# xandergos/terrain-diffusion

Hardware: AMD Instinct MI355X
Metric: terrain megapixels/sec (decoded) at fixed steps, 30m model (higher is better)
Workload: dtype bf16; 1 GPU; BASELINE configs[2]: terrain-diffusion-30m base U-Net, 8x8 tile grid (stride 32, 288x288 latents) with overlap blending, 20 steps, 64 windows batched per solver step; edm_steps=20, parallelism=1 independent streams (one process per GPU, no data-path collective)

## Files before the change

### terrain_diffusion_amd/csrc/conv_common.h

```cpp
#pragma once
#include "td_device.h"

#ifdef TD_ABLATE_BLOAD
#define TD_ABL_BLOAD(X)
#else
#define TD_ABL_BLOAD(X) X
#endif
#ifdef TD_ABLATE_BARRIER
#define TD_ABL_BARRIER(X)
#else
#define TD_ABL_BARRIER(X) X
#endif
#ifdef TD_ABLATE_BSTORE
#define TD_ABL_BSTORE(X)
#else
#define TD_ABL_BSTORE(X) X
#endif

#define TD_SWZ(r) (((r) >> 1) & 7)

namespace td {

typedef __bf16 bf16x8 __attribute__((ext_vector_type(8)));
typedef __bf16 bf16x4 __attribute__((ext_vector_type(4)));
// ... 244 lines not shown
            const f32x2 r[4] = {{(float)ra[0], (float)ra[1]}, {(float)ra[2], (float)ra[3]}, {(float)rb[0], (float)rb[1]}, {(float)rb[2], (float)rb[3]}};
#pragma unroll
            for (int q = 0; q < 4; ++q) v[q] = v[q] + rs * r[q];
        }
        if (clip > 0.f) {
#pragma unroll
            for (int q = 0; q < 4; ++q) v[q] = f32x2{__builtin_amdgcn_fmed3f(v[q].x, -clip, clip), __builtin_amdgcn_fmed3f(v[q].y, -clip, clip)};
        }
    }
    const hx4 ha = {(T)v[0].x, (T)v[0].y, (T)v[1].x, (T)v[1].y};
    const hx4 hb = {(T)v[2].x, (T)v[2].y, (T)v[3].x, (T)v[3].y};
    const f32x2 f[4] = {{(float)ha[0], (float)ha[1]}, {(float)ha[2], (float)ha[3]}, {(float)hb[0], (float)hb[1]}, {(float)hb[2], (float)hb[3]}};
    if (want_ss) {
        f32x2 s2 = f[0] * f[0];
#pragma unroll
        for (int q = 1; q < 4; ++q) s2 = f[q] * f[q] + s2;
        ss += s2.x + s2.y;
    }
    {
        const u32x2 pa = __builtin_bit_cast(u32x2, ha), pb = __builtin_bit_cast(u32x2, hb);
        unsigned a0 = pa[0], a1 = pa[1], b0 = pb[0], b1 = pb[1];
        swap_halves(a0, b0); swap_halves(a1, b1);
        o = u32x4{a0, a1, b0, b1};
    }
    if (want_o2) {
        f32x2 g[4];
#pragma unroll
        for (int q = 0; q < 4; ++q) g[q] = silu_k2(f[q], k_o2);
        const hx4 ga = {(T)g[0].x, (T)g[0].y, (T)g[1].x, (T)g[1].y}, gb = {(T)g[2].x, (T)g[2].y, (T)g[3].x, (T)g[3].y};
        const u32x2 qa = __builtin_bit_cast(u32x2, ga), qb = __builtin_bit_cast(u32x2, gb);
        unsigned c0 = qa[0], c1 = qa[1], d0 = qb[0], d1 = qb[1];
        swap_halves(c0, d0); swap_halves(c1, d1);
        o2 = u32x4{c0, c1, d0, d1};
    }
}

template <int TW, int TPIX>
__device__ __forceinline__ void frag_pixel(int q0, int l31, int& img, int& ty, int& tx) {
#ifndef TD_NO_REMAP
#define TD_REMAP_ON 1
#else
#define TD_REMAP_ON 0
#endif
    if constexpr (TW == 16 && TD_REMAP_ON) {
        const bool g2 = (l31 >= 4 && l31 < 12) || (l31 >= 16 && l31 < 20) || l31 >= 28;
        const int u = g2 ? (l31 < 12 ? l31 - 4 : (l31 < 20 ? l31 - 8 : l31 - 16)) : (l31 < 4 ? l31 : (l31 < 16 ? l31 - 8 : l31 - 12));
        img = q0 / TPIX;
        ty = (q0 % TPIX) / 16 + (g2 ? 1 : 0);
        tx = u;
    } else if constexpr (TW == 8 && TD_REMAP_ON) {
        const bool g2 = (l31 >= 4 && l31 < 12) || (l31 >= 16 && l31 < 20) || l31 >= 28;
        const int u = g2 ? (l31 < 12 ? l31 - 4 : (l31 < 20 ? l31 - 8 : l31 - 16)) : (l31 < 4 ? l31 : (l31 < 16 ? l31 - 8 : l31 - 12));
        img = q0 / TPIX;
        ty = (q0 % TPIX) / 8 + (u >> 2);
        tx = (u & 3) + (g2 ? 4 : 0);
    } else {
        const int q = q0 + l31, r = q % TPIX;
        img = q / TPIX; ty = r / TW; tx = r % TW;
    }
}

}
```

### terrain_diffusion_amd/csrc/engine.hip

```cpp
#include <hip/hip_runtime.h>
#include <math.h>
#include <stdio.h>
#include <string.h>

#include <map>
#include <memory>
#include <string>
#include <vector>
#include <unordered_map>

#include "../../include/td_engine.h"
#include "td_device.h"

#include "conv_igemm.hip"
#include "conv_glds.hip"
#include "conv_glds_wide.hip"
#include "conv_sb.hip"
#include "conv_s16.hip"
#include "conv_fewcout.hip"
#include "small_kernels.hip"
#include "compose_kernels.hip"
#include "attn_mfma.hip"

using namespace td;

#define TD_DISPATCH_T(U, ...)                                                       \
    do {                                                                             \
        if ((U)->dt == TD_DTYPE_BF16) { typedef __bf16 T_; __VA_ARGS__; }            \
        else if ((U)->dt == TD_DTYPE_F16) { typedef _Float16 T_; __VA_ARGS__; }      \
        else { typedef float T_; __VA_ARGS__; }                                      \
    } while (0)

static thread_local std::string g_err;
static int fail(int code, const std::string& msg) { g_err = msg; return code; }
#define HIP_TRY(expr)                                                                                      \
    do {                                                                                                   \
        hipError_t _e = (expr);                                                                            \
        if (_e != hipSuccess) return fail(TD_ERR_HIP, std::string(#expr) + ": " + hipGetErrorString(_e)); \
    } while (0)

static inline uint16_t f2h(float f) {
    _Float16 h = (_Float16)f;
    uint16_t u;
    memcpy(&u, &h, 2);
    return u;
}
static inline uint16_t f2bf(float f) {
    uint32_t u;
    memcpy(&u, &f, 4);
// ... 185 lines not shown
    bool set = false;
    int64_t numel() const { int64_t n = 1; for (int i = 0; i < ndim; ++i) n *= shape[i]; return n; }
};

struct WSeg {
    const std::vector<float>* w = nullptr;
    int cin_tot = 0, cin_off = 0, c_real = 0, c_pad = 0, taps = 9;
    float mul = 1.f;
};
struct ConvWeights {
    std::vector<WSeg> segs;
    int cout = 0, cout_pad = 0;
    Buf packed;
    int ksteps = 0;
    Buf packed_sb;
    size_t packed_bytes = 0;
    Buf packed_s16;
    int sb_n3 = 0, sb_g1 = 0;
};

struct Tensor {
    void* ptr = nullptr;
    int C = 0, cstride = 0, H = 0, W = 0;
    float* sumsq = nullptr;
    int nparts = 0;
};

struct Op {
    enum Kind { CONV, ATTN } kind = CONV;
    ConvParams p;
    bool narrow = false;
    int bn = 64;
    int glds_variant = 0;
    int flavor = 0;
    int sb_mt = 2, sb_nt = 2;
    int cvec_off = -1;
    double k_alg = 0.0;
    int out_C = 0, out_H = 0, out_W = 0;
    const void* qkv = nullptr; void* att = nullptr; int tokens = 0, C = 0;
    void* attn_ws = nullptr;
    std::string label;
};

struct Plan {
    int N = 0, H = 0, W = 0;
    std::vector<Op> ops;
    std::vector<Buf> bufs;
    void* xin = nullptr;
    float* F = nullptr;
    float* partial = nullptr;
    Buf x, m1, m2, xt, cond, emb, cvec, tsteps;
    int cvec_rows = 0;
    int cvec_written = 0;
    hipGraphExec_t graph = nullptr;
    std::vector<float> graph_sigmas;
    float graph_sigma_data = 0.f;
    int graph_solver_order = 0;
    int graph_lof = -1;
    int graph_fuse = -1;
    int graph_stop = -2;
    const void* graph_guide = nullptr;
    const void* graph_guide_cvec = nullptr;
    float graph_gscale = 0.f;
    float graph_alpha = 1.f;
    std::vector<float> graph_cs;
    size_t bytes = 0;
// ... 297 lines not shown
            if ((rc = mk(n + ".conv_res1", b.cout, s1))) return rc;
        }
        if (b.attn) {
            if ((rc = mk(n + ".attn_qkv", 3 * b.cout, {seg(n + ".attn_qkv.weight", 1.f, b.cout, 0, b.cout, 1, 1.f)}))) return rc;
            if ((rc = mk(n + ".attn_proj", b.cout, {seg(n + ".attn_proj.weight", 1.f, b.cout, 0, b.cout, 1, kMixNew)}))) return rc;
        }
        return TD_OK;
    };
    for (auto& b : u->enc) if ((rc = do_block(b))) return rc;
    for (auto& b : u->dec) if ((rc = do_block(b))) return rc;
    if ((rc = mk("out_conv", u->cfg.out_channels, {seg("out_conv.weight", out_gain, u->final_c, 0, u->final_c, 9, 1.f)}))) return rc;
    for (auto& p : u->params) { p.data.clear(); p.data.shrink_to_fit(); }
    u->folded.clear();
    HIP_TRY(hipDeviceSynchronize());
    u->finalized = true;
    return TD_OK;
}

static int new_buf(Plan& pl, size_t bytes, void** out) {
    Buf b(new DevBuf());
    HIP_TRY(b->alloc(bytes, true));
    *out = b->p;
    pl.bytes += b->bytes;
    pl.bufs.push_back(std::move(b));
    return TD_OK;
}

struct SegSpec { const Tensor* t; int C; int taps; int resample; int xform; float scale; };

static int build_plan(td_unet* u, int N, int H, int W, Plan** out, int lane = 0) {
    static const char* const kPlanOptions[] = {"batch_invariant", "glds", "splitk", "producer_act", "glds_min_wgs", "glds_variant", "glds_bn",
                                               "glds_splitk", "glds_splitk_max", "glds_splitk_min_groups", "splitk_target_wgs",
                                               "bn128_min_wgs", "attn_mfma", "glds_splitk_from_groups", "glds_bn64", "glds_small_max_groups", "glds_round_aware", "walk_alternate", "glds_tiny", "glds_dma1x1", "splitk_weighted",
                                               "sb", "sb_target_wgs", "sb_mt", "sb_nt", "sb_order", "sb_max_glds_wgs", "sb_splitk", "sb_splitk_wgs", "sb_splitk_max", "s16", "s16_min_wgs", "sb_m4", "glds_wide", "glds_wide_min_wgs", "glds_wide_tail", "glds_wide_persist", "fewcout"};
    std::string key = std::to_string(N) + "_" + std::to_string(H) + "_" + std::to_string(W);
    for (const char* o : kPlanOptions) key += "_" + std::to_string((long long)u->eng->option(o, -7));
    if (lane) key += "_lane" + std::to_string(lane);
    auto it = u->plans.find(key);
    if (it != u->plans.end()) { it->second->last_use = ++u->use_clock; *out = it->second.get(); return TD_OK; }
    if (N < 1 || N > 1023 || H > 1023 || W > 1023) return fail(TD_ERR_ARG, "batch/size out of range");
    const int down = 1 << (u->cfg.n_levels - 1);
    if (H % down || W % down) return fail(TD_ERR_ARG, "H and W must be divisible by 2^(levels-1)");
    {
        const size_t budget = (size_t)u->eng->option("plan_cache_mb", 65536) << 20;
        const size_t max_plans = (size_t)u->eng->option("plan_cache_max", 12);
        size_t total = 0;
        for (auto& kv : u->plans) total += kv.second->bytes;
        while (!u->plans.empty() && (total > budget || u->plans.size() >= max_plans)) {
            auto victim = u->plans.begin();
            for (auto jt = u->plans.begin(); jt != u->plans.end(); ++jt) if (jt->second->last_use < victim->second->last_use) victim = jt;
            HIP_TRY(hipStreamSynchronize(u->eng->stream));
            total -= victim->second->bytes;
            u->plans.erase(victim);
        }
    }
    std::unique_ptr<Plan> plp(new Plan());
    Plan& pl = *plp;
    pl.N = N; pl.H = H; pl.W = W;
    const size_t es = u->esize();
    const int chunk = u->chunk;
    const bool use_splitk = u->eng->option("splitk", 1) != 0;
    const int64_t splitk_target = u->eng->option("splitk_target_wgs", 512);
    const int64_t bn128_min = u->eng->option("bn128_min_wgs", 128);
    int rc;
    size_t partial_bytes = 0;

    auto new_tensor = [&](int C, int h, int w, bool want_sumsq, int nparts, Tensor* t) -> int {
// ... 62 lines not shown
            if (u->bf16 && bn2 && u->eng->option("glds", 1) && (inv || sb_takes || mt2 * (cw.cout_pad / bn2) >= u->eng->option("glds_min_wgs", 8))) {
                op.flavor = 2; op.bn = bn2; op.glds_variant = variant;
                int TH2 = variant ? 8 : (op.narrow ? 8 : 16);
                const int NIMG2 = op.narrow ? (variant ? 2 : 4) : 1;
                p.tiles_x = (w + TW2 - 1) / TW2; p.tiles_y = (h + TH2 - 1) / TH2; p.img_groups = (N + NIMG2 - 1) / NIMG2;
                p.n_ntiles = cw.cout_pad / bn2; p.ksplit = 1;
                const int64_t wgs = mt2 * p.n_ntiles, slots = variant ? 512 : 256;
                const bool may_split = !inv && use_splitk && u->eng->option("glds_splitk", 1) && wgs * 2 <= slots;
                if (may_split && kgroups >= u->eng->option("glds_splitk_from_groups", 2))
                    p.ksplit = (int)std::min<int64_t>(std::min<int64_t>(u->eng->option("glds_splitk_max", 32), kgroups / std::max<int64_t>(1, u->eng->option("glds_splitk_min_groups", 1))), slots / wgs);
                if (may_split && !op.narrow && variant == 1 && u->eng->option("glds_tiny", 0) != 0) {
                    const int64_t wgs_tiny = tiles(4, 1) * (cw.cout_pad / 64);
                    if (wgs_tiny <= 384) {
                        op.glds_variant = 2; op.bn = 64; TH2 = 4;
                        p.tiles_y = (h + TH2 - 1) / TH2; p.n_ntiles = cw.cout_pad / 64;
                        p.ksplit = (int)std::max<int64_t>(1, std::min<int64_t>(std::min<int64_t>(kgroups, u->eng->option("glds_splitk_max", 32)), 384 / wgs_tiny));
                    }
                }
                {
                    const int64_t wmode = u->eng->option("glds_wide", 1);
                    const int bnw = cw.cout_pad % 96 == 0 ? 96 : (cw.cout_pad % 64 == 0 ? 64 : 0);
                    const int64_t tmode = u->eng->option("glds_wide_tail", 1);
                    bool pure3 = true;
                    for (const SegSpec& sg : segs) if (sg.taps != 9 && (sg.xform != 0 || tmode == 0 || (tmode == 1 && bnw != 64))) pure3 = false;
                    const int64_t wgs_w = bnw ? tiles(16, 1) * (cw.cout_pad / bnw) : 0;
                    if (wmode != 0 && !inv && fv < 0 && fbn == 0 && !op.narrow && p.ksplit == 1 && bnw && !out_f32 && (cw.cout & 7) == 0 && p.nseg <= 3 && (pure3 || wmode == 2) &&
                        (wmode == 2 || wgs_w >= u->eng->option("glds_wide_min_wgs", 384))) {
                        op.glds_variant = 3; op.bn = bnw;
                        p.tiles_x = (w + 15) / 16; p.tiles_y = (h + 15) / 16; p.img_groups = N; p.n_ntiles = cw.cout_pad / bnw;
                        bool tail3 = false;
                        for (const SegSpec& sg : segs) if (sg.taps != 9) tail3 = true;
                        if (u->eng->option("glds_wide_persist", 0) != 0 && bnw == 64 && !tail3 && (h & 15) == 0 && (w & 15) == 0 && cw.cout == cw.cout_pad)
                            p.persist = conv_wide_persist_grid((long long)p.tiles_x * p.tiles_y * N * p.n_ntiles, 2 * std::max(1, u->eng->n_cus));
                    }
                }
                if (op.flavor == 2 && sb_takes && op.glds_variant != 3) {
                    {
                        const int TWs = op.narrow ? 8 : 16;
                        auto th_of = [&](int mt) { return op.narrow ? (mt == 2 ? 8 : 4) : (mt == 4 ? 8 : mt == 2 ? 4 : 2); };
                        auto sb_wgs = [&](int mt, int nt) { return (int64_t)((w + TWs - 1) / TWs) * ((h + th_of(mt) - 1) / th_of(mt)) * N * (cw.cout_pad / (32 * nt)); };
                        const int64_t target = u->eng->option("sb_target_wgs", 160);
                        int mt = 1, nt = 1, ks = 1;
                        if (!op.narrow && u->eng->option("sb_m4", 0) != 0 && sb_wgs(2, 2) >= target && sb_wgs(4, 1) >= target) { mt = 4; nt = 1; }
                        else if (sb_wgs(2, 2) >= target) { mt = 2; nt = 2; } else if (sb_wgs(2, 1) >= target) { mt = 2; nt = 1; }
                        else if (use_splitk && u->eng->option("sb_splitk", 1) != 0 && sb_wgs(2, 1) * 2 <= u->eng->option("sb_splitk_wgs", 224)) {
                            mt = 2; nt = 1;
                            ks = (int)std::min<int64_t>(std::min<int64_t>(kgroups, u->eng->option("sb_splitk_max", 16)), (u->eng->option("sb_splitk_wgs", 224) + sb_wgs(2, 1) / 2) / sb_wgs(2, 1));
                        }
                        const int64_t fmt = u->eng->option("sb_mt", 0), fnt = u->eng->option("sb_nt", 0);
                        if (fmt == 1 || fmt == 2 || (fmt == 4 && !op.narrow)) { mt = (int)fmt; ks = 1; }
                        if (fnt == 1 || fnt == 2) { nt = (int)fnt; ks = 1; if (mt == 4 && fnt == 2 && fmt != 4) mt = 2; }
                        if (mt == 4) nt = 1;
                        const int64_t s16_mode = u->eng->option("s16", 1);
                        const int64_t wgs16 = sb_wgs(2, 1) * 2;
                        const bool s16 = s16_mode == 2 || (s16_mode == 1 && fmt == 0 && fnt == 0 && sb_wgs(2, 2) < target && sb_wgs(2, 1) < target &&
                                                           wgs16 <= u->eng->option("sb_splitk_wgs", 224) && wgs16 >= u->eng->option("s16_min_wgs", 128));
                        if (s16) {
                            if ((rc = ensure_packed_s16(u, cw))) return rc;
                            op.flavor = 5; op.sb_mt = 2; op.sb_nt = 0; p.ksplit = 1;
                            p.tiles_x = (w + TWs - 1) / TWs; p.tiles_y = (h + th_of(2) - 1) / th_of(2); p.img_groups = N; p.n_ntiles = cw.cout_pad / 16;
                            p.wpack_sb = cw.packed_s16->p; p.sb_n3 = cw.sb_n3;
                        } else {
                        if ((rc = ensure_packed_sb(u, cw))) return rc;
                        op.flavor = 4; op.sb_mt = mt; op.sb_nt = nt; p.ksplit = ks < 1 ? 1 : ks;
                        p.tiles_x = (w + TWs - 1) / TWs; p.tiles_y = (h + th_of(mt) - 1) / th_of(mt); p.img_groups = N; p.n_ntiles = cw.cout_pad / (32 * nt);
                        p.wpack_sb = cw.packed_sb->p; p.sb_n3 = cw.sb_n3;
// ... 255 lines not shown
                if (kind[i / 2] == 0) { u->eng->prof_conv_ms += ms; u->eng->prof_conv_launches++; } else { u->eng->prof_other_ms += ms; u->eng->prof_other_launches++; }
            }
            for (auto e : evs) (void)hipEventDestroy(e);
        }
    } fin{u, evs, ev_kind, ev_label, ev_flop, st};
    for (auto& op : pl.ops) {
        if (op.kind == Op::ATTN) {
            mark();
            if (op.attn_ws) {
                const int Hh = op.C / 64, L = op.tokens;
                size_t qn, kn, vn;
                attn_workspace_elems(pl.N, Hh, L, L, 64, &qn, &kn, &vn);
                __bf16 *Qp = (__bf16*)op.attn_ws, *Kp = Qp + qn, *Vt = Kp + kn;
                const __bf16* qkv = (const __bf16*)op.qkv;
                const AttnStrides so = {(long)L * op.C, 64L, (long)op.C, 1L};
                hipError_t ea = attn_pack_qkv64<__bf16>(qkv, 3L * op.C, pl.N, Hh, L, 0.125f, Qp, Kp, Vt, st);
                if (ea == hipSuccess) ea = attn_mfma(Qp, Kp, Vt, nullptr, (__bf16*)op.att, so, pl.N, Hh, L, L, 64, st);
                if (ea != hipSuccess) return fail(TD_ERR_HIP, std::string("attention launch: ") + hipGetErrorString(ea));
            } else
            TD_DISPATCH_T(u, hipLaunchKernelGGL(attn_kernel<T_>, dim3(pl.N, op.C / 64), dim3(256), 0, st, (const T_*)op.qkv, (T_*)op.att, op.tokens, op.C));
            mark(); if (prof) { ev_kind.push_back(1); ev_label.push_back(op.label); ev_flop.push_back(0.0); }
            HIP_TRY(hipGetLastError());
            continue;
        }
        ConvParams p = op.p;
        if (op.cvec_off >= 0) p.cvec = cbase + op.cvec_off;
        if (fuse && &op == &pl.ops.back()) {
            p.epi = EPI_DPM_STEP; p.dpm_x = (float*)pl.x->p; p.dpm_m1 = (float*)pl.m1->p; p.dpm_m2 = u->eng->option("solver_order", 2) == 3 ? (float*)pl.m2->p : nullptr; p.dpm_xin = pl.xin; p.dpm_xin_cstride = u->chunk; p.dpm_k = *fuse;
        }
        mark();
        hipError_t e = op.flavor == 6 ? launch_conv_fewcout(p, u->dt, st)
                       : op.flavor == 5 ? launch_conv_s16(p, u->dt, op.narrow, st)
                       : op.flavor == 4 ? launch_conv_sb(p, u->dt, op.narrow, op.sb_mt, op.sb_nt, st)
                       : op.flavor == 2 ? (op.glds_variant == 3 ? launch_conv_glds_wide(p, u->dt, op.bn, st) : launch_conv_glds(p, u->dt, op.narrow, op.bn, op.glds_variant, st))
                       : launch_conv(p, u->dt, op.narrow, op.bn, 0, st);
        mark(); if (prof) { ev_kind.push_back(0); char tag[160]; double gf_ = op.k_alg * 2.0 * p.N * p.H * p.W * p.Cout * 1e-9;
            double mb_ = 0.0; const double es_ = (double)u->esize();
            for (int si_ = 0; si_ < p.nseg; ++si_) mb_ += (double)p.N * p.seg[si_].Hs * p.seg[si_].Ws * p.seg[si_].C * es_ + (double)p.seg[si_].C / 64.0 * p.seg[si_].taps * p.CoutPad * 128.0 * (es_ / 2.0);
            if (p.res) mb_ += (double)p.N * p.res_Hs * p.res_Ws * p.Cout * es_;
            const double o1_ = (double)p.N * p.H * p.W * p.Cout * (p.out_f32 ? 4.0 : es_);
            const double mbs_ = (mb_ + o1_) * 1e-6;
            mb_ += o1_ * (p.out2 ? 2.0 : 1.0);
            mb_ *= 1e-6;
            snprintf(tag, sizeof tag, " [%dx%d k%d f%d%s bn%d wg%d ks%d gf%.2f mb%.2f mbs%.2f]", p.H, p.W, p.kgroups, op.flavor, op.flavor == 5 ? "c16" : op.flavor == 4 ? (op.sb_mt == 4 ? "m4n1" : op.sb_mt == 2 ? (op.sb_nt == 2 ? "m2n2" : "m2n1") : (op.sb_nt == 2 ? "m1n2" : "m1n1")) : op.flavor == 2 ? (op.glds_variant == 3 ? (p.persist > 0 ? "wp" : "w") : op.glds_variant == 2 ? "t" : op.glds_variant ? "s" : "b") : "", op.bn, p.n_ntiles * p.tiles_x * p.tiles_y * p.img_groups, p.ksplit, gf_, mb_, mbs_); ev_label.push_back(op.label + tag);
            ev_flop.push_back(op.flavor == 2 ? 2.0 * p.N * p.H * p.W * (double)p.Cout * op.k_alg : 0.0); }
        if (e != hipSuccess) return fail(TD_ERR_HIP, "conv launch " + op.label + ": " + hipGetErrorString(e));
    }
    return TD_OK;
}

static inline dim3 grid1(size_t n, int b = 256) { return dim3((unsigned)((n + b - 1) / b)); }

extern "C" {

const char* td_last_error(void) { return g_err.c_str(); }
int td_version(void) { return 1; }
#ifndef TD_CSRC_SHA
#define TD_CSRC_SHA "unstamped"
#endif
const char* td_build_id(void) { return TD_CSRC_SHA; }

int td_engine_create(int device_id, td_engine** out) {
    if (!out) return fail(TD_ERR_ARG, "null out");
    int ndev = 0;
    if (hipGetDeviceCount(&ndev) != hipSuccess || ndev == 0) return fail(TD_ERR_HIP, "no HIP device visible: the engine has no CPU fallback");
    if (device_id < 0 || device_id >= ndev) return fail(TD_ERR_ARG, "bad device id");
    DevGuard dg_(device_id);
    td_engine* e = new td_engine();
    e->device = device_id;
    { hipDeviceProp_t prop; if (hipGetDeviceProperties(&prop, device_id) == hipSuccess && prop.multiProcessorCount > 0) e->n_cus = prop.multiProcessorCount; }
    hipError_t err = hipStreamCreateWithFlags(&e->stream, hipStreamNonBlocking);
    e->own_stream = e->stream;
    if (err == hipSuccess) err = hipStreamCreateWithFlags(&e->stream2, hipStreamNonBlocking);
    if (err == hipSuccess) err = hipEventCreateWithFlags(&e->ev_fork, hipEventDisableTiming);
    if (err == hipSuccess) err = hipEventCreateWithFlags(&e->ev_join, hipEventDisableTiming);
    if (err == hipSuccess) err = hipMalloc(&e->zeros, 4096);
    if (err == hipSuccess) err = hipMemset(e->zeros, 0, 4096);
    if (err == hipSuccess) err = hipDeviceSynchronize();
    if (err != hipSuccess) { if (e->stream) (void)hipStreamDestroy(e->stream); if (e->stream2) (void)hipStreamDestroy(e->stream2); if (e->ev_fork) (void)hipEventDestroy(e->ev_fork); if (e->ev_join) (void)hipEventDestroy(e->ev_join); delete e; return fail(TD_ERR_HIP, hipGetErrorString(err)); }
    *out = e;
    return TD_OK;
}
void td_engine_destroy(td_engine* e) {
    if (!e) return;
    DevGuard dg_(e->device);
    if (e->own_stream) { (void)hipStreamSynchronize(e->stream); (void)hipStreamDestroy(e->own_stream); }
    if (e->stream2) (void)hipStreamDestroy(e->stream2);
    if (e->ev_fork) (void)hipEventDestroy(e->ev_fork);
    if (e->ev_join) (void)hipEventDestroy(e->ev_join);
    if (e->zeros) (void)hipFree(e->zeros);
    delete e;
}
int td_engine_synchronize(td_engine* e) {
    DevGuard dg_(e->device); HIP_TRY(hipStreamSynchronize(e->stream)); e->deferred.clear(); e->ring.reset(); return TD_OK; }
void* td_engine_stream(td_engine* e) { return (void*)e->stream; }
int td_engine_set_stream(td_engine* e, void* hip_stream) {
    if (!e) return fail(TD_ERR_ARG, "null engine");
    DevGuard dg_(e->device);
    HIP_TRY(hipStreamSynchronize(e->stream));
    e->deferred.clear();
    e->ring.reset();
    e->stream = hip_stream ? (hipStream_t)hip_stream : e->own_stream;
    return TD_OK;
}
static const char* const kKnownOptions[] = {
    "async", "batch_invariant", "fuse_solver", "graph", "lower_order_final", "profile", "solver_order", "dual_stream", "dual_stream_min_batch", "sampler_stop_after",
    "plan_cache_mb", "plan_cache_max", "grid_fused",
    "attn_mfma", "bn128_min_wgs", "glds", "glds_bn", "glds_bn64", "glds_dma1x1", "glds_min_wgs", "glds_round_aware", "glds_small_max_groups",
    "glds_splitk", "glds_splitk_from_groups", "glds_splitk_max", "glds_splitk_min_groups", "glds_tiny", "glds_variant", "glds_wide", "glds_wide_min_wgs", "glds_wide_tail", "glds_wide_persist", "fewcout",
    "producer_act", "s16", "s16_min_wgs", "sb", "sb_m4", "sb_max_glds_wgs", "sb_mt", "sb_nt", "sb_order", "sb_splitk", "sb_splitk_max", "sb_splitk_wgs", "sb_target_wgs", "splitk",
    "splitk_target_wgs", "splitk_weighted", "walk_alternate"};
int td_engine_set_option(td_engine* e, const char* key, int64_t value) {
    if (!e || !key) return fail(TD_ERR_ARG, "null");
    bool known = false;
    for (const char* k : kKnownOptions) known = known || strcmp(k, key) == 0;
    if (!known) return fail(TD_ERR_ARG, std::string("unknown engine option \"") + key + "\" (include/td_engine.h lists the options)");
    e->opt[key] = value;
    return TD_OK;
}

int64_t td_engine_get_option(td_engine* e, const char* key, int64_t dflt) { return (e && key) ? e->option(key, dflt) : dflt; }

int td_engine_profile_read(td_engine* e, double* conv_ms, int64_t* conv_launches, double* other_ms, int64_t* other_launches, int reset) {
    if (conv_ms) *conv_ms = e->prof_conv_ms;
    if (conv_launches) *conv_launches = e->prof_conv_launches;
    if (other_ms) *other_ms = e->prof_other_ms;
    if (other_launches) *other_launches = e->prof_other_launches;
    if (reset) { e->prof_conv_ms = e->prof_other_ms = 0.0; e->prof_conv_launches = e->prof_other_launches = 0; e->prof_ops.clear(); }
    return TD_OK;
}
int td_engine_profile_read_glds(td_engine* e, double* ms, double* flop, int64_t* launches, int reset) {
    if (ms) *ms = e->prof_glds_ms;
    if (flop) *flop = e->prof_glds_flop;
    if (launches) *launches = e->prof_glds_launches;
    if (reset) { e->prof_glds_ms = e->prof_glds_flop = 0.0; e->prof_glds_launches = 0; }
    return TD_OK;
}
int td_engine_profile_dump(td_engine* e, char* buf, int64_t capacity) {
    std::string out;
    for (auto& kv : e->prof_ops) {
        char line[256];
        snprintf(line, sizeof line, "%s\t%.4f\t%lld\n", kv.first.c_str(), kv.second.first, (long long)kv.second.second);
// ... 882 lines not shown
```

Measured before the change: 21.96 MP/s.

## Add 16x16 MFMA wide conv kernel for BN=96 pure 3x3 layers

Adds a new implicit-GEMM 3x3 conv kernel for the wide GLDS path that uses 16x16x(k) MFMA fragments over 16x16 pixel tiles with an 18x18 LDS halo patch, a 4-slot weight DMA ring, and a new epilogue variant that skips the half-swap shuffle. It is enabled by default for BN=96 non-persistent layers without 1x1 tails. The aim is better MFMA utilisation and a different tile/operand layout than the existing wide kernel. It adds a large new kernel with its own addressing and layout, which carries correctness risk and shifts register and LDS pressure.

```diff
diff --git a/terrain_diffusion_amd/csrc/conv_common.h b/terrain_diffusion_amd/csrc/conv_common.h
--- a/terrain_diffusion_amd/csrc/conv_common.h
+++ b/terrain_diffusion_amd/csrc/conv_common.h
@@ -300,6 +300,51 @@
         unsigned c0 = qa[0], c1 = qa[1], d0 = qb[0], d1 = qb[1];
         swap_halves(c0, d0); swap_halves(c1, d1);
         o2 = u32x4{c0, c1, d0, d1};
+    }
+}
+
+template <typename T>
+__device__ __forceinline__ void epi_unit8n(int epi, bool has_res, float clip, bool want_ss, bool want_o2, f32x4 va, f32x4 vb, f32x4 ca, f32x4 cb, u32x4 rw,
+                                           float rs, SiluK k_o2, u32x4& o, u32x4& o2, float& ss) {
+    typedef typename Half<T>::x4 hx4;
+    f32x2 v[4] = {{va[0], va[1]}, {va[2], va[3]}, {vb[0], vb[1]}, {vb[2], vb[3]}};
+    if (epi == EPI_EMB_SILU) {
+        const f32x2 c[4] = {{ca[0], ca[1]}, {ca[2], ca[3]}, {cb[0], cb[1]}, {cb[2], cb[3]}};
+        const SiluK k = silu_k(1.f);
+#pragma unroll
+        for (int q = 0; q < 4; ++q) v[q] = silu_k2(v[q] * c[q], k);
+    } else if (epi == EPI_RESIDUAL) {
+        if (has_res) {
+            const hx4 ra = __builtin_bit_cast(hx4, u32x2{rw[0], rw[1]}), rb = __builtin_bit_cast(hx4, u32x2{rw[2], rw[3]});
+            const f32x2 r[4] = {{(float)ra[0], (float)ra[1]}, {(float)ra[2], (float)ra[3]}, {(float)rb[0], (float)rb[1]}, {(float)rb[2], (float)rb[3]}};
+#pragma unroll
+            for (int q = 0; q < 4; ++q) v[q] = v[q] + rs * r[q];
+        }
+        if (clip > 0.f) {
+#pragma unroll
+            for (int q = 0; q < 4; ++q) v[q] = f32x2{__builtin_amdgcn_fmed3f(v[q].x, -clip, clip), __builtin_amdgcn_fmed3f(v[q].y, -clip, clip)};
+        }
+    }
+    const hx4 ha = {(T)v[0].x, (T)v[0].y, (T)v[1].x, (T)v[1].y};
+    const hx4 hb = {(T)v[2].x, (T)v[2].y, (T)v[3].x, (T)v[3].y};
+    const f32x2 f[4] = {{(float)ha[0], (float)ha[1]}, {(float)ha[2], (float)ha[3]}, {(float)hb[0], (float)hb[1]}, {(float)hb[2], (float)hb[3]}};
+    if (want_ss) {
+        f32x2 s2 = f[0] * f[0];
+#pragma unroll
+        for (int q = 1; q < 4; ++q) s2 = f[q] * f[q] + s2;
+        ss += s2.x + s2.y;
+    }
+    {
+        const u32x2 pa = __builtin_bit_cast(u32x2, ha), pb = __builtin_bit_cast(u32x2, hb);
+        o = u32x4{pa[0], pa[1], pb[0], pb[1]};
+    }
+    if (want_o2) {
+        f32x2 g[4];
+#pragma unroll
+        for (int q = 0; q < 4; ++q) g[q] = silu_k2(f[q], k_o2);
+        const hx4 ga = {(T)g[0].x, (T)g[0].y, (T)g[1].x, (T)g[1].y}, gb = {(T)g[2].x, (T)g[2].y, (T)g[3].x, (T)g[3].y};
+        const u32x2 qa = __builtin_bit_cast(u32x2, ga), qb = __builtin_bit_cast(u32x2, gb);
+        o2 = u32x4{qa[0], qa[1], qb[0], qb[1]};
     }
 }
 
diff --git a/terrain_diffusion_amd/csrc/conv_glds_wide16.hip b/terrain_diffusion_amd/csrc/conv_glds_wide16.hip
--- /dev/null
+++ b/terrain_diffusion_amd/csrc/conv_glds_wide16.hip
@@ -0,0 +1,408 @@
+#include "conv_common.h"
+
+namespace td {
+
+#ifdef TD_TRACE
+#define TDX_T(v) unsigned long long v = __builtin_amdgcn_s_memtime(); asm volatile("s_waitcnt lgkmcnt(0)" ::: "memory")
+#define TDX_TACC(acc, a, b) acc += (b) - (a)
+#else
+#define TDX_T(v)
+#define TDX_TACC(acc, a, b)
+#endif
+
+__device__ __forceinline__ void w16_pixel(int wave, int i, int lane, int& ty, int& tx) {
+    const int n = lane & 15;
+    const bool s2 = n >= 4 && n < 12;
+    const int k = s2 ? n - 4 : (n < 4 ? n : n - 8);
+    ty = wave * 4 + (i >> 1) * 2 + (s2 ? 1 : 0);
+    tx = 2 * k + (i & 1);
+}
+
+template <typename T>
+__global__ __launch_bounds__(256, 2) void conv_glds_kernel_x16(const ConvParams p) {
+    typedef typename Half<T>::x8 hx8;
+    constexpr int BN = 96;
+    constexpr int NTHR = 256, TH = 16, TW = 16;
+    constexpr int PW = 18, NPATCH = 18 * 18;
+    constexpr int MB = 4, NB = BN / 16, NP = BN / 32;
+    constexpr int CHUNK = 64, HALF = 32, PER16 = 8;
+    constexpr int A_ITERS = (NPATCH * 4 + NTHR - 1) / NTHR;
+    constexpr int A_FULL = NPATCH * 4 / NTHR, A_REM = NPATCH * 4 - A_FULL * NTHR;
+    constexpr int NBI = 2;
+    constexpr int H_BYTES = BN * 64, RING = 4;
+    constexpr int DUMP_BASE = RING * H_BYTES;
+    constexpr int PITCH = 80;
+    constexpr int A_BASE = DUMP_BASE + 2048, A_BYTES = NPATCH * PITCH;
+    constexpr int RN_BASE = A_BASE + 2 * A_BYTES, RN_BYTES = (NPATCH * 4 + 15) / 16 * 16;
+    constexpr int CV_BASE = RN_BASE + RN_BYTES;
+    constexpr int NUNIT = MB * NP;
+    static_assert(2 * A_BYTES + 2 * PW * PITCH + 2 * PITCH + (2 * PW + 1) * PITCH + 64 < 65536, "ds_read offset field");
+    static_assert(A_REM < NTHR && A_ITERS == A_FULL + 1, "patch pieces");
+
+    extern __shared__ __attribute__((aligned(16))) unsigned char smem[];
+    float* s_rn = (float*)(smem + RN_BASE);
+    float* s_cv = (float*)(smem + CV_BASE);
+
+    const int tid = threadIdx.x, lane = tid & 63, wave = __builtin_amdgcn_readfirstlane(tid >> 6);
+    const int lg = lane >> 4;
+#ifdef TD_TRACE
+    unsigned long long tr_wait = 0, tr_stage = 0;
+#endif
+    TDX_T(tr_start);
+#ifdef TD_TRACE
+    const unsigned long long tr_rt0 = __builtin_amdgcn_s_memrealtime();
+#endif
+
+    unsigned k_d1 = p.sb_d1, k_m1 = p.sb_m1, k_m2 = p.sb_m2, k_m3 = p.sb_m3, k_g8 = p.sb_grid8, k_grid = p.sb_grid;
+    int k_tx = p.tiles_x, k_ty = p.tiles_y, k_rev = p.reverse, k_cpad = p.CoutPad, k_N = p.N, k_H = p.H, k_W = p.W;
+    const unsigned char* k_wpack = (const unsigned char*)p.wpack;
+    int k_epi = p.epi, k_Cout = p.Cout, k_cvs = p.cvec_stride;
+    int k_c0 = p.seg[0].C, k_c1 = p.seg[1].C, k_c2 = p.seg[2].C, k_t0 = p.seg[0].taps, k_t1 = p.seg[1].taps, k_t2 = p.seg[2].taps;
+    const bool k_hres = p.res != nullptr;
+    asm volatile("" : "+s"(k_cpad), "+s"(k_N), "+s"(k_H), "+s"(k_W), "+s"(k_wpack), "+s"(k_epi), "+s"(k_Cout), "+s"(k_cvs));
+    int n0, y0, x0, co0;
+    {
+        unsigned ubid = blockIdx.x;
+        if (k_g8) ubid = (ubid & 7) * k_g8 + (ubid >> 3);
+        if (k_rev) ubid = k_grid - 1 - ubid;
+        const unsigned mtile = td_udiv(ubid, k_d1, k_m1);
+        const int ntile = (int)(ubid - mtile * k_d1);
+        const unsigned q2 = td_udiv(mtile, (unsigned)k_tx, k_m2);
+        const int txi = (int)(mtile - q2 * (unsigned)k_tx), ig = (int)td_udiv(q2, (unsigned)k_ty, k_m3), tyi = (int)(q2 - (unsigned)ig * (unsigned)k_ty);
+        n0 = ig; y0 = tyi * TH; x0 = txi * TW; co0 = ntile * BN;
+    }
+    const int u0 = k_t0 == 9 ? k_c0 / CHUNK : 0, u1 = (k_t0 == 9 && k_t1 == 9) ? k_c1 / CHUNK : 0, u2 = (u1 > 0 && k_t2 == 9) ? k_c2 / CHUNK : 0;
+    const int n3 = u0 + u1 + u2;
+
+    const size_t wstep = (size_t)k_cpad * 128;
+    const unsigned char* wchunk = k_wpack + (size_t)co0 * 128;
+    const unsigned char* wnext = wchunk;
+    unsigned wvoff[NBI];
+#pragma unroll
+    for (int i = 0; i < NBI; ++i) {
+        const int pos = tid + i * NTHR, b = (pos >> 6) % NB, m = pos & 15, j = (pos >> 4) & 3;
+        const int r = (b >> 1) * 32 + (m >> 2) * 8 + (b & 1) * 4 + (m & 3), x = TD_SWZ(r);
+        wvoff[i] = (unsigned)(r * 128 + ((((x & 4) | (j ^ (x & 3)))) << 4));
+    }
+    const unsigned ldsw = (unsigned)wave * 1024u;
+    const bool dump1 = wave >= 2;
+    const unsigned voff1 = dump1 ? wvoff[0] : wvoff[1];
+    unsigned wslot = 0, rslot = 0;
+#define TDX_SLOT_NEXT(X) { X += H_BYTES; if (X == RING * H_BYTES) X = 0; }
+#define TDX_DMA(TILE)                                                                                        \
+    {                                                                                                        \
+        if ((TILE) == 9) wnext = wchunk;                                                                     \
+        if ((TILE) == 18) { wnext += wstep; wchunk = wnext; }                                                \
+        const unsigned x_ = ((TILE) >= 9 && (TILE) < 18) ? 64u : 0u;                                         \
+        { const unsigned v_ = wvoff[0] ^ x_; const unsigned m_ = ldsw + wslot; TD_GLDS16(v_, wnext, m_, 0); } \
+        { const unsigned v_ = voff1 ^ x_; const unsigned m_ = dump1 ? (unsigned)DUMP_BASE + ldsw - 2048u : ldsw + wslot + 4096u; TD_GLDS16(v_, wnext, m_, 0); } \
+        TDX_SLOT_NEXT(wslot)                                                                                 \
+        if ((TILE) != 8 && (TILE) != 17) wnext += wstep;                                                     \
+    }
+    TDX_DMA(0); TDX_DMA(1); TDX_DMA(2);
+    const bool cv_stage = k_epi == EPI_EMB_SILU && tid < BN;
+    float cv_val = 0.f;
+    if (cv_stage) {
+        if (n0 < k_N && co0 + tid < k_Cout) cv_val = p.cvec[(size_t)n0 * k_cvs + co0 + tid];
+    }
+
+    u32x4 av[A_ITERS];
+    int aoff[A_ITERS];
+    const T* seg_src = nullptr;
+    int seg_xform = 0, seg_nchunks = 0;
+    float seg_scale = 1.f;
+#define TDX_SEG_BEGIN(SEG)                                                                                            \
+    {                                                                                                                 \
+        seg_src = (const T*)p.seg[SEG].src; seg_xform = p.seg[SEG].xform; seg_scale = p.seg[SEG].scale; seg_nchunks = p.seg[SEG].C / CHUNK; \
+        const int Hs_ = p.seg[SEG].Hs, Ws_ = p.seg[SEG].Ws, rs_ = p.seg[SEG].resample, cs_ = p.seg[SEG].cstride;      \
+        _Pragma("unroll") for (int it_ = 0; it_ < A_ITERS; ++it_) {                                                   \
+            int e_ = tid + it_ * NTHR;                                                                                \
+            asm volatile("" : "+v"(e_));    \
+            const int pp_ = e_ >> 2, py_ = pp_ / PW, px_ = pp_ - py_ * PW;                                            \
+            const int y_ = y0 + py_ - 1, x_ = x0 + px_ - 1;                                                           \
+            const bool ok_ = pp_ < NPATCH && n0 < k_N && y_ >= 0 && y_ < k_H && x_ >= 0 && x_ < k_W;                  \
+            aoff[it_] = -1;                                                                                           \
+            if (ok_) aoff[it_] = src_pixel(n0, y_, x_, Hs_, Ws_, rs_) * cs_ + (e_ & 3) * PER16;                      \
+        }                                                                                                             \
+    }
+#define TDX_LOAD_A(CH, HF)                                                                             \
+    {                                                                                                  \
+        const T* src_ = seg_src + (CH) * CHUNK + (HF) * HALF;                                          \
+        _Pragma("unroll") for (int it_ = 0; it_ < A_ITERS; ++it_) {                                    \
+            const unsigned o_ = (unsigned)(aoff[it_] >= 0 ? aoff[it_] : 0) * (unsigned)sizeof(T);      \
+            asm volatile(TD_SGPR_GUARD_LOAD "global_load_dwordx4 %0, %1, %2" : "=&v"(av[it_]) : "v"(o_), "s"(src_) : "memory"); \
+        }                                                                                              \
+    }
+#define TDX_PIN_A() { _Pragma("unroll") for (int it_ = 0; it_ < A_ITERS; ++it_) asm volatile("" : "+v"(av[it_])); }
+    const unsigned st_base = (unsigned)A_BASE + (unsigned)(tid >> 2) * PITCH + (unsigned)((tid & 3) << 4);
+#define TDX_STORE_A(BUF)                                                                               \
+    {                                                                                                  \
+        _Pragma("unroll") for (int it_ = 0; it_ < A_ITERS; ++it_) {                                    \
+            if (it_ < A_FULL || tid < A_REM) {                                                         \
+                u32x4 v_ = aoff[it_] >= 0 ? av[it_] : u32x4{0u, 0u, 0u, 0u};                           \
+                if (seg_xform != 0 && aoff[it_] >= 0) {                                                \
+                    float s_ = seg_scale;                                                              \
+                    if (seg_xform == 2) s_ *= s_rn[(tid >> 2) + it_ * (NTHR / 4)];                     \
+                    v_ = xform_piece<T>(v_, s_);                                                       \
+                }                                                                                      \
+                *(u32x4*)(smem + st_base + ((BUF) * A_BYTES + it_ * (NTHR / 4) * PITCH)) = v_;         \
+            }                                                                                          \
+        }                                                                                              \
+    }
+    const bool r_want = k_epi == EPI_RESIDUAL && k_hres;
+    bool r_pref = false;
+#define TDX_R_PTR(I, DST)                                                                                             \
+    {                                                                                                                 \
+        int ty_, tx_; ln_ = tid;                                                                                      \
+        asm volatile("" : "+v"(ln_));    \
+        w16_pixel(ln_ >> 6, I, ln_, ty_, tx_);                                                                          \
+        const int y_ = y0 + ty_, x_ = x0 + tx_;                                                                       \
+        const int sp_ = (n0 < k_N && y_ < k_H && x_ < k_W) ? src_pixel(n0, y_, x_, p.res_Hs, p.res_Ws, p.res_resample) : 0; \
+        DST = (const T*)p.res + ((size_t)sp_ * p.res_cstride + co0 + 8 * ((ln_ >> 4) & 3));                           \
+    }
+#define TDX_R_OFF(Q) ((co0 + ((Q) % NP) * 32 + 8 * ((ln_ >> 4) & 3) < k_Cout) ? ((Q) % NP) * 32 : 0)
+#define TDX_LOAD_R()                                                                                                  \
+    {                                                                                                                 \
+        _Pragma("unroll") for (int i_ = 0; i_ < (A_ITERS + NP - 1) / NP; ++i_) {                                      \
+            const T* rp_; int ln_; TDX_R_PTR(i_, rp_)                                                                 \
+            _Pragma("unroll") for (int j_ = 0; j_ < NP; ++j_) if (i_ * NP + j_ < A_ITERS) av[i_ * NP + j_] = *(const u32x4*)(rp_ + TDX_R_OFF(i_ * NP + j_)); \
+        }                                                                                                             \
+        r_pref = true;                                                                                                \
+    }
+    TDX_SEG_BEGIN(0);
+    TDX_LOAD_A(0, 0);
+
+    unsigned xbase;
+    {
+        int ty, tx;
+        w16_pixel(tid >> 6, 0, lane, ty, tx);
+        xbase = (unsigned)A_BASE + (unsigned)(ty * PW + tx) * PITCH + (unsigned)lg * 16u;
+    }
+    const unsigned wbase = (unsigned)lane * 16u;
+
+    {
+        const float* rn_sumsq = nullptr; int rn_parts = 0, rn_Hs = 0, rn_Ws = 0, rn_res = 0; float rn_invc = 0.f;
+        if (p.seg[0].xform == 2) { rn_sumsq = p.seg[0].sumsq; rn_parts = p.seg[0].nparts; rn_Hs = p.seg[0].Hs; rn_Ws = p.seg[0].Ws; rn_res = p.seg[0].resample; rn_invc = p.seg[0].inv_c; }
+        else if (p.res_sumsq) { rn_sumsq = p.res_sumsq; rn_parts = p.res_nparts; rn_Hs = p.res_Hs; rn_Ws = p.res_Ws; rn_res = p.res_resample; rn_invc = p.res_inv_c; }
+        if (rn_sumsq) {
+            const size_t npix = (size_t)k_N * rn_Hs * rn_Ws;
+            for (int pp = tid; pp < NPATCH; pp += NTHR) {
+                const int py = pp / PW, px = pp % PW;
+                const int y = y0 + py - 1, x = x0 + px - 1;
+                float rn = 0.f;
+                if (n0 < k_N && y >= 0 && y < k_H && x >= 0 && x < k_W)
+                    rn = pixel_rn(rn_sumsq, rn_parts, npix, src_pixel(n0, y, x, rn_Hs, rn_Ws, rn_res), rn_invc);
+                s_rn[pp] = rn;
+            }
+        }
+    }
+    {
+        int t_ = tid, e_ = k_epi;
+        asm volatile("" : "+v"(t_), "+s"(e_));
+        if (e_ == EPI_EMB_SILU && t_ < BN) s_cv[t_] = cv_val;
+    }
+
+    __syncthreads();
+    asm volatile("s_waitcnt vmcnt(0)" ::: "memory");
+    { TDX_PIN_A() TDX_STORE_A(0); }
+    f32x4 acc[MB][NB];
+#pragma unroll
+    for (int i = 0; i < MB; ++i)
+#pragma unroll
+        for (int b = 0; b < NB; ++b) acc[i][b] = f32x4{0.f, 0.f, 0.f, 0.f};
+    TDX_T(tr_pro);
+
+#define TDX_TOFF(TP) ((((TP) / 3) * PW + ((TP) % 3)) * PITCH)
+#define TDX_XOFF(I) ((((I) >> 1) * 2 * PW + ((I) & 1)) * PITCH)
+    u32x4 wf_[NB], xf_[2][MB];
+#define TDX_READ_W(B0, B1, SLOT) { _Pragma("unroll") for (int b_ = (B0); b_ < (B1); ++b_) wf_[b_] = *(const u32x4*)(smem + (wbase + (SLOT)) + b_ * 1024); }
+#define TDX_READ_X(XP, BUF, TOFF) { _Pragma("unroll") for (int i_ = 0; i_ < MB; ++i_) xf_[XP][i_] = *(const u32x4*)(smem + xbase + ((BUF) * A_BYTES + (TOFF) + TDX_XOFF(i_))); }
+#define TDX_MFMA(B0, B1, XP)                                                                                \
+    {                                                                                                        \
+        _Pragma("unroll") for (int b_ = (B0); b_ < (B1); ++b_)                                               \
+            _Pragma("unroll") for (int i_ = 0; i_ < MB; ++i_)                                                \
+                acc[i_][b_] = Half<T>::mfma16(__builtin_bit_cast(hx8, wf_[b_]), __builtin_bit_cast(hx8, xf_[XP][i_]), acc[i_][b_]); \
+    }
+#define TDX_HS(S)                                                                                            \
+    {                                                                                                        \
+        TDX_T(tA_);                                                                                          \
+         \
+        if ((S) == 1 || (S) == 2 || (((S) == 10 || (S) == 11) && nxt)) asm volatile("s_waitcnt vmcnt(%0)" ::"n"(A_ITERS + NBI) : "memory"); \
+        else if ((S) >= 16 && !nxt) { if (r_now) asm volatile("s_waitcnt vmcnt(%0)" ::"n"(A_ITERS) : "memory"); else asm volatile("s_waitcnt vmcnt(0)" ::: "memory"); } \
+        else asm volatile("s_waitcnt vmcnt(%0)" ::"n"(NBI) : "memory");                                      \
+        if ((S) == 6 || (S) == 15) asm volatile("s_waitcnt lgkmcnt(0)" ::: "memory");    \
+        TDX_T(tM_); TDX_TACC(tr_stage, tA_, tM_);                                                            \
+        __builtin_amdgcn_s_barrier();                                                                        \
+        asm volatile("" ::: "memory");                                                                       \
+        TDX_T(tB_); TDX_TACC(tr_wait, tA_, tB_);                                                             \
+        if ((S) == 3 || ((S) == 12 && nxt)) TDX_PIN_A()    \
+        if ((S) + 3 < 18 || nxt) TDX_DMA((S) + 3);    \
+        if ((S) == 0) TDX_LOAD_A(chunk, 1);                                                                  \
+        if ((S) == 9 && nxt) { if (newseg) TDX_SEG_BEGIN(seg + 1); TDX_LOAD_A(newseg ? 0 : chunk + 1, 0); }  \
+        if ((S) == 15 && r_now) TDX_LOAD_R()                                                                 \
+        if ((S) == 5) TDX_STORE_A(1);                                                                        \
+        if ((S) == 14 && nxt) TDX_STORE_A(0);                                                                \
+        TDX_MFMA(0, NB / 2, (S) & 1);                                                                        \
+        if ((S) < 17 || nxt) { TDX_READ_X(((S) + 1) & 1, (((S) + 1) / 9) & 1, TDX_TOFF(((S) + 1) % 9)); TDX_READ_W(0, NB / 2, rslot); } \
+        TDX_MFMA(NB / 2, NB, (S) & 1);                                                                       \
+        if ((S) < 17 || nxt) { TDX_READ_W(NB / 2, NB, rslot); TDX_SLOT_NEXT(rslot) }                         \
+        __builtin_amdgcn_sched_group_barrier(0x008, MB * NB / 2, 0);                                         \
+        __builtin_amdgcn_sched_group_barrier(0x100, MB + NB / 2, 0);                                         \
+        __builtin_amdgcn_sched_group_barrier(0x008, MB * NB / 2, 0);                                         \
+        __builtin_amdgcn_sched_group_barrier(0x100, NB / 2, 0);                                              \
+    }
+    int seg = 0, chunk = 0;
+    if (n3 > 0) {
+        asm volatile("s_waitcnt vmcnt(%0)" ::"n"(2 * NBI) : "memory");
+        asm volatile("s_waitcnt lgkmcnt(0)" ::: "memory");
+        __builtin_amdgcn_s_barrier();
+        asm volatile("" ::: "memory");
+        TDX_READ_X(0, 0, TDX_TOFF(0));
+        TDX_READ_W(0, NB, rslot);
+        TDX_SLOT_NEXT(rslot)
+    }
+    for (int u = 0; u < n3; ++u) {
+        const bool last = u + 1 == n3;
+        const bool nxt = !last;
+        const bool newseg = !last && chunk + 1 == seg_nchunks;
+        const bool r_now = r_want && last;
+        TDX_HS(0); TDX_HS(1); TDX_HS(2); TDX_HS(3); TDX_HS(4); TDX_HS(5); TDX_HS(6); TDX_HS(7); TDX_HS(8);
+        TDX_HS(9); TDX_HS(10); TDX_HS(11); TDX_HS(12); TDX_HS(13); TDX_HS(14); TDX_HS(15); TDX_HS(16); TDX_HS(17);
+        if (newseg) { ++seg; chunk = 0; } else ++chunk;
+    }
+    asm volatile("s_waitcnt vmcnt(0)" ::: "memory");
+    TDX_T(tr_loop);
+
+    int e_Cout = p.Cout, e_epi = p.epi, e_ocs = p.out_cstride;
+    float e_rsc = p.res_scale, e_clip = p.clip, e_o2s = p.out2_scale;
+    const bool e_hres = p.res != nullptr, e_hrss = p.res_sumsq != nullptr, e_hoss = p.out_sumsq != nullptr, e_ho2 = p.out2 != nullptr;
+    asm volatile("" : "+s"(e_Cout), "+s"(e_epi), "+s"(e_ocs), "+s"(e_rsc), "+s"(e_clip), "+s"(e_o2s), "+s"(co0));
+    const size_t M = (size_t)k_N * k_H * k_W;
+    int elane = tid;
+    asm volatile("" : "+v"(elane));
+    const int elg = (elane >> 4) & 3;
+    const bool has_res = e_epi == EPI_RESIDUAL && e_hres;
+    constexpr int NRX = NUNIT - A_ITERS;
+    u32x4 rx[NRX];
+#pragma unroll
+    for (int q = 0; q < NRX; ++q) rx[q] = u32x4{0u, 0u, 0u, 0u};
+    if (has_res) {
+        if (!r_pref) TDX_LOAD_R()
+#pragma unroll
+        for (int i = A_ITERS / NP; i < MB; ++i) {
+            const T* rp; int ln_; TDX_R_PTR(i, rp)
+#pragma unroll
+            for (int j = 0; j < NP; ++j) rx[i * NP + j - A_ITERS] = *(const u32x4*)(rp + TDX_R_OFF(i * NP + j));
+        }
+    }
+    static_assert(A_ITERS % NP == 0, "the prefetched residual runs are whole pixel blocks");
+#pragma unroll
+    for (int i = 0; i < MB; ++i) {
+        int ty, tx;
+        w16_pixel(elane >> 6, i, elane, ty, tx);
+        const int n = n0, y = y0 + ty, x = x0 + tx;
+        const bool ok = n < k_N && y < k_H && x < k_W;
+        float ssj[NP];
+#pragma unroll
+        for (int j = 0; j < NP; ++j) ssj[j] = 0.f;
+        const size_t pix = ((size_t)n * k_H + y) * k_W + x;
+        if (ok) {
+            const float rn = e_hrss ? s_rn[(ty + 1) * PW + (tx + 1)] : 1.f;
+            T* orow = (T*)p.out + pix * e_ocs + co0 + 8 * elg;
+            const float rs = e_rsc * rn;
+            const bool want_ss = e_hoss, want_o2 = e_ho2;
+            const SiluK k_o2 = silu_k(e_o2s);
+            auto body = [&](auto KIND) __attribute__((always_inline)) {
+                constexpr int K = decltype(KIND)::value;
+#pragma unroll
+                for (int j = 0; j < NP; ++j) {
+                    f32x4 ca = {0.f, 0.f, 0.f, 0.f}, cb = ca;
+                    u32x4 rw = {0u, 0u, 0u, 0u};
+                    if constexpr (K == 1) {
+                        const float* c_ = s_cv + j * 32 + 8 * elg;
+                        ca = *(const f32x4*)c_; cb = *(const f32x4*)(c_ + 4);
+                    }
+                    if constexpr (K == 2) rw = i * NP + j < A_ITERS ? av[i * NP + j < A_ITERS ? i * NP + j : 0] : rx[i * NP + j >= A_ITERS ? i * NP + j - A_ITERS : 0];
+                    u32x4 o, o2;
+                    epi_unit8n<T>(e_epi, has_res, e_clip, want_ss, want_o2, acc[i][2 * j], acc[i][2 * j + 1], ca, cb, rw, rs, k_o2, o, o2, ssj[j]);
+                    if (co0 + j * 32 + 8 * elg < e_Cout) {
+                        *(u32x4*)(orow + j * 32) = o;
+                        if (want_o2) *(u32x4*)((T*)p.out2 + (orow - (T*)p.out) + j * 32) = o2;
+                    } else ssj[j] = 0.f;
+                }
+            };
+            if (e_epi == EPI_EMB_SILU) body(std::integral_constant<int, 1>{});
+            else if (has_res) body(std::integral_constant<int, 2>{});
+            else body(std::integral_constant<int, 0>{});
+        }
+        if (e_hoss) {
+#pragma unroll
+            for (int j = 0; j < NP; ++j) {
+                float ss = ssj[j] + __shfl_xor(ssj[j], 16);
+                ss += __shfl_xor(ss, 32);
+                if (ok && elg == 0 && co0 + j * 32 < k_cpad) p.out_sumsq[(size_t)((unsigned)co0 / 32u + j) * M + pix] = ss;
+            }
+        }
+    }
+#undef TDX_TOFF
+#undef TDX_XOFF
+#undef TDX_HS
+#undef TDX_READ_W
+#undef TDX_READ_X
+#undef TDX_MFMA
+#undef TDX_LOAD_A
+#undef TDX_PIN_A
+#undef TDX_STORE_A
+#undef TDX_SEG_BEGIN
+#undef TDX_DMA
+#undef TDX_SLOT_NEXT
+#undef TDX_R_PTR
+#undef TDX_R_OFF
+#undef TDX_LOAD_R
+#ifdef TD_TRACE
+    TDX_T(tr_eissue);
+    asm volatile("s_waitcnt vmcnt(0)" ::: "memory");
+    TDX_T(tr_end);
+    if (lane == 0) {
+        unsigned long long* tb = (unsigned long long*)p.partial + ((size_t)blockIdx.x * 4 + wave) * 16;
+        tb[0] = tr_pro - tr_start; tb[1] = tr_loop - tr_pro; tb[2] = tr_end - tr_loop; tb[3] = tr_wait; tb[4] = tr_stage; tb[5] = tr_start; tb[6] = tr_end;
+        tb[8] = tr_rt0; tb[9] = ((unsigned long long)__builtin_amdgcn_s_getreg((31 << 11) | 4) << 8) | __builtin_amdgcn_s_getreg((3 << 11) | 20);
+        tb[10] = __builtin_amdgcn_s_memrealtime();
+        tb[7] = tb[10] - tr_rt0; tb[11] = tr_end - tr_eissue;
+    }
+#endif
+}
+
+template <typename T>
+static hipError_t launch_glds_wide16_cfg(const ConvParams& p, hipStream_t st) {
+    constexpr int BN = 96, NPATCH = 18 * 18;
+    constexpr size_t LDS = 4 * (size_t)(BN * 64) + 2048 + 2 * (size_t)NPATCH * 80 + (size_t)(NPATCH * 4 + 15) / 16 * 16 + (size_t)BN * 4;
+    static_assert(2 * LDS <= 160 * 1024, "two workgroups per CU");
+    if (p.ksplit != 1 || p.persist != 0 || p.W < 16 || p.CoutPad % BN || p.nseg < 1 || p.nseg > 3 || p.kgroups < 1) return hipErrorInvalidValue;
+    if (p.out_f32 || (p.Cout & 7) || p.epi == EPI_DPM_STEP) return hipErrorInvalidValue;
+    int units = 0;
+    for (int s = 0; s < p.nseg; ++s) { if (p.seg[s].taps != 9 || p.seg[s].C % 64) return hipErrorInvalidValue; units += p.seg[s].C / 64; }
+    if (units != p.kgroups) return hipErrorInvalidValue;
+    ConvParams pd = p;
+    for (int s = p.nseg; s < 3; ++s) { pd.seg[s].C = 0; pd.seg[s].taps = 0; }
+    const int mtiles = p.tiles_x * p.tiles_y * p.img_groups, grid = p.n_ntiles * mtiles;
+    if (grid <= 0 || (long long)grid * std::max(mtiles, p.n_ntiles) >= ((long long)1 << 32)) return hipErrorInvalidValue;
+    pd.sb_d0 = mtiles; pd.sb_m0 = td_magic(mtiles); pd.sb_d1 = p.n_ntiles; pd.sb_m1 = td_magic(p.n_ntiles); pd.sb_m2 = td_magic(p.tiles_x); pd.sb_m3 = td_magic(p.tiles_y);
+    pd.sb_grid = grid; pd.sb_grid8 = (grid & 7) == 0 ? (unsigned)grid >> 3 : 0u;
+    auto kern = conv_glds_kernel_x16<T>;
+    static bool attr_set[64] = {};
+    int dev_ = 0; (void)hipGetDevice(&dev_);
+    if (dev_ < 0 || dev_ >= 64 || !attr_set[dev_]) {
+        hipError_t e = hipFuncSetAttribute((const void*)kern, hipFuncAttributeMaxDynamicSharedMemorySize, (int)LDS);
+        if (e != hipSuccess) return e;
+        if (dev_ >= 0 && dev_ < 64) attr_set[dev_] = true;
+    }
+    hipLaunchKernelGGL(kern, dim3(grid), dim3(256), LDS, st, pd);
+    return hipGetLastError();
+}
+
+hipError_t launch_conv_glds_wide16(const ConvParams& p, int dtype, hipStream_t st) {
+    return dtype == 2 ? launch_glds_wide16_cfg<_Float16>(p, st) : launch_glds_wide16_cfg<__bf16>(p, st);
+}
+
+}
diff --git a/terrain_diffusion_amd/csrc/engine.hip b/terrain_diffusion_amd/csrc/engine.hip
--- a/terrain_diffusion_amd/csrc/engine.hip
+++ b/terrain_diffusion_amd/csrc/engine.hip
@@ -15,6 +15,7 @@
 #include "conv_igemm.hip"
 #include "conv_glds.hip"
 #include "conv_glds_wide.hip"
+#include "conv_glds_wide16.hip"
 #include "conv_sb.hip"
 #include "conv_s16.hip"
 #include "conv_fewcout.hip"
@@ -266,6 +267,7 @@
     bool narrow = false;
     int bn = 64;
     int glds_variant = 0;
+    bool wide16 = false;
     int flavor = 0;
     int sb_mt = 2, sb_nt = 2;
     int cvec_off = -1;
@@ -629,7 +631,7 @@
     static const char* const kPlanOptions[] = {"batch_invariant", "glds", "splitk", "producer_act", "glds_min_wgs", "glds_variant", "glds_bn",
                                                "glds_splitk", "glds_splitk_max", "glds_splitk_min_groups", "splitk_target_wgs",
                                                "bn128_min_wgs", "attn_mfma", "glds_splitk_from_groups", "glds_bn64", "glds_small_max_groups", "glds_round_aware", "walk_alternate", "glds_tiny", "glds_dma1x1", "splitk_weighted",
-                                               "sb", "sb_target_wgs", "sb_mt", "sb_nt", "sb_order", "sb_max_glds_wgs", "sb_splitk", "sb_splitk_wgs", "sb_splitk_max", "s16", "s16_min_wgs", "sb_m4", "glds_wide", "glds_wide_min_wgs", "glds_wide_tail", "glds_wide_persist", "fewcout"};
+                                               "sb", "sb_target_wgs", "sb_mt", "sb_nt", "sb_order", "sb_max_glds_wgs", "sb_splitk", "sb_splitk_wgs", "sb_splitk_max", "s16", "s16_min_wgs", "sb_m4", "glds_wide", "glds_wide_min_wgs", "glds_wide_tail", "glds_wide_persist", "glds_wide_mfma16", "fewcout"};
     std::string key = std::to_string(N) + "_" + std::to_string(H) + "_" + std::to_string(W);
     for (const char* o : kPlanOptions) key += "_" + std::to_string((long long)u->eng->option(o, -7));
     if (lane) key += "_lane" + std::to_string(lane);
@@ -758,6 +760,7 @@
                         for (const SegSpec& sg : segs) if (sg.taps != 9) tail3 = true;
                         if (u->eng->option("glds_wide_persist", 0) != 0 && bnw == 64 && !tail3 && (h & 15) == 0 && (w & 15) == 0 && cw.cout == cw.cout_pad)
                             p.persist = conv_wide_persist_grid((long long)p.tiles_x * p.tiles_y * N * p.n_ntiles, 2 * std::max(1, u->eng->n_cus));
+                        op.wide16 = u->eng->option("glds_wide_mfma16", 1) != 0 && bnw == 96 && !tail3 && p.persist == 0;
                     }
                 }
                 if (op.flavor == 2 && sb_takes && op.glds_variant != 3) {
@@ -1079,7 +1082,7 @@
         hipError_t e = op.flavor == 6 ? launch_conv_fewcout(p, u->dt, st)
                        : op.flavor == 5 ? launch_conv_s16(p, u->dt, op.narrow, st)
                        : op.flavor == 4 ? launch_conv_sb(p, u->dt, op.narrow, op.sb_mt, op.sb_nt, st)
-                       : op.flavor == 2 ? (op.glds_variant == 3 ? launch_conv_glds_wide(p, u->dt, op.bn, st) : launch_conv_glds(p, u->dt, op.narrow, op.bn, op.glds_variant, st))
+                       : op.flavor == 2 ? (op.glds_variant == 3 ? (op.wide16 ? launch_conv_glds_wide16(p, u->dt, st) : launch_conv_glds_wide(p, u->dt, op.bn, st)) : launch_conv_glds(p, u->dt, op.narrow, op.bn, op.glds_variant, st))
                        : launch_conv(p, u->dt, op.narrow, op.bn, 0, st);
         mark(); if (prof) { ev_kind.push_back(0); char tag[160]; double gf_ = op.k_alg * 2.0 * p.N * p.H * p.W * p.Cout * 1e-9;
             double mb_ = 0.0; const double es_ = (double)u->esize();
@@ -1089,7 +1092,7 @@
             const double mbs_ = (mb_ + o1_) * 1e-6;
             mb_ += o1_ * (p.out2 ? 2.0 : 1.0);
             mb_ *= 1e-6;
-            snprintf(tag, sizeof tag, " [%dx%d k%d f%d%s bn%d wg%d ks%d gf%.2f mb%.2f mbs%.2f]", p.H, p.W, p.kgroups, op.flavor, op.flavor == 5 ? "c16" : op.flavor == 4 ? (op.sb_mt == 4 ? "m4n1" : op.sb_mt == 2 ? (op.sb_nt == 2 ? "m2n2" : "m2n1") : (op.sb_nt == 2 ? "m1n2" : "m1n1")) : op.flavor == 2 ? (op.glds_variant == 3 ? (p.persist > 0 ? "wp" : "w") : op.glds_variant == 2 ? "t" : op.glds_variant ? "s" : "b") : "", op.bn, p.n_ntiles * p.tiles_x * p.tiles_y * p.img_groups, p.ksplit, gf_, mb_, mbs_); ev_label.push_back(op.label + tag);
+            snprintf(tag, sizeof tag, " [%dx%d k%d f%d%s bn%d wg%d ks%d gf%.2f mb%.2f mbs%.2f%s]", p.H, p.W, p.kgroups, op.flavor, op.flavor == 5 ? "c16" : op.flavor == 4 ? (op.sb_mt == 4 ? "m4n1" : op.sb_mt == 2 ? (op.sb_nt == 2 ? "m2n2" : "m2n1") : (op.sb_nt == 2 ? "m1n2" : "m1n1")) : op.flavor == 2 ? (op.glds_variant == 3 ? (p.persist > 0 ? "wp" : "w") : op.glds_variant == 2 ? "t" : op.glds_variant ? "s" : "b") : "", op.bn, p.n_ntiles * p.tiles_x * p.tiles_y * p.img_groups, p.ksplit, gf_, mb_, mbs_, (op.flavor == 2 && op.glds_variant == 3 && op.wide16) ? " x16" : ""); ev_label.push_back(op.label + tag);
             ev_flop.push_back(op.flavor == 2 ? 2.0 * p.N * p.H * p.W * (double)p.Cout * op.k_alg : 0.0); }
         if (e != hipSuccess) return fail(TD_ERR_HIP, "conv launch " + op.label + ": " + hipGetErrorString(e));
     }
@@ -1154,7 +1157,7 @@
     "async", "batch_invariant", "fuse_solver", "graph", "lower_order_final", "profile", "solver_order", "dual_stream", "dual_stream_min_batch", "sampler_stop_after",
     "plan_cache_mb", "plan_cache_max", "grid_fused",
     "attn_mfma", "bn128_min_wgs", "glds", "glds_bn", "glds_bn64", "glds_dma1x1", "glds_min_wgs", "glds_round_aware", "glds_small_max_groups",
-    "glds_splitk", "glds_splitk_from_groups", "glds_splitk_max", "glds_splitk_min_groups", "glds_tiny", "glds_variant", "glds_wide", "glds_wide_min_wgs", "glds_wide_tail", "glds_wide_persist", "fewcout",
+    "glds_splitk", "glds_splitk_from_groups", "glds_splitk_max", "glds_splitk_min_groups", "glds_tiny", "glds_variant", "glds_wide", "glds_wide_min_wgs", "glds_wide_tail", "glds_wide_persist", "glds_wide_mfma16", "fewcout",
     "producer_act", "s16", "s16_min_wgs", "sb", "sb_m4", "sb_max_glds_wgs", "sb_mt", "sb_nt", "sb_order", "sb_splitk", "sb_splitk_max", "sb_splitk_wgs", "sb_target_wgs", "splitk",
     "splitk_target_wgs", "splitk_weighted", "walk_alternate"};
 int td_engine_set_option(td_engine* e, const char* key, int64_t value) {
```

Result: faster. 22.33 MP/s, median of 6 (+1.7%).
